# caki35/UNet-Torch

Hardware: AMD Instinct MI355X
Metric: images/sec training step, 4-level U-Net 1ch→2cls 512×512, at 1/2/4/8 MI355X (higher is better)
Workload: dtype f16

## Files before the change

unet-torch_amd/csrc/stem_head.hip:

```cpp
#include "kernels.h"

typedef _Float16 half8 __attribute__((ext_vector_type(8)));

namespace {

constexpr int STEM_PPB = 1024;
constexpr int WG_PPB = 4096;

inline bool al16(const void* p) { return (((uintptr_t)p) & 15) == 0; }

template <int CI>
__global__ __launch_bounds__(256) void stem3x3_fwd_kernel(const half_t* __restrict__ x, int ldx,
                                                          const float4* __restrict__ tx, const half_t* __restrict__ wp,
                                                          half_t* __restrict__ y, int ldy, float* __restrict__ part,
                                                          int N, int H, int W, int Co) {
    extern __shared__ __attribute__((aligned(16))) float sm[];
    const int tid = threadIdx.x;
    const int G = Co >> 3, PL = 256 / G;
    const int cg = tid % G, pl = tid / G;
    float* wsm = sm;
    for (int i = tid; i < 9 * CI * Co; i += 256) wsm[i] = (float)wp[i];
    __syncthreads();
    const long P = (long)N * H * W;
    const long p0 = (long)blockIdx.x * STEM_PPB;
    float s[8], q[8];
#pragma unroll
    for (int j = 0; j < 8; ++j) s[j] = q[j] = 0.f;
    const int RUN = STEM_PPB / PL;
    long p = p0 + (long)pl * RUN;
    long pend = p + RUN;
    if (pend > P) pend = P;
    if (pend > p0 + STEM_PPB) pend = p0 + STEM_PPB;
    int n = 0, yy = 0, xx = 0;
    if (p < pend) {
        n = (int)(p / ((long)H * W));
        const int r = (int)(p - (long)n * H * W);
        yy = r / W;
        xx = r - yy * W;
    }
    float win[3][3][CI];
    bool fresh = true;
    for (; p < pend; ++p) {
#pragma unroll
        for (int dy = 0; dy < 3; ++dy) {
            const int hi = yy + dy - 1;
            const bool rowok = hi >= 0 && hi < H;
            const half_t* xr = x + ((long)((long)n * H + (rowok ? hi : 0)) * W) * ldx;
#pragma unroll
            for (int dx = 0; dx < 3; ++dx) {
                if (!fresh && dx < 2) {
#pragma unroll
                    for (int ci = 0; ci < CI; ++ci) win[dy][dx][ci] = win[dy][dx + 1][ci];
                    continue;
                }
                const int wi = xx + dx - 1;
                const bool ok = rowok && wi >= 0 && wi < W;
#pragma unroll
                for (int ci = 0; ci < CI; ++ci) {
                    float v = 0.f;
                    if (ok) {
                        v = (float)xr[(long)wi * ldx + ci];
                        if (tx) v = umi_tx(v, tx[ci]);
                    }
                    win[dy][dx][ci] = v;
                }
            }
        }
        fresh = false;
        float acc[8];
#pragma unroll
        for (int j = 0; j < 8; ++j) acc[j] = 0.f;
#pragma unroll
        for (int tap = 0; tap < 9; ++tap)
#pragma unroll
            for (int ci = 0; ci < CI; ++ci) {
                const float v = win[tap / 3][tap % 3][ci];
                const float4* wrow = reinterpret_cast<const float4*>(wsm + (tap * CI + ci) * Co + cg * 8);
                float4 w0 = wrow[0], w1 = wrow[1];
                acc[0] = fmaf(v, w0.x, acc[0]); acc[1] = fmaf(v, w0.y, acc[1]);
                acc[2] = fmaf(v, w0.z, acc[2]); acc[3] = fmaf(v, w0.w, acc[3]);
                acc[4] = fmaf(v, w1.x, acc[4]); acc[5] = fmaf(v, w1.y, acc[5]);
                acc[6] = fmaf(v, w1.z, acc[6]); acc[7] = fmaf(v, w1.w, acc[7]);
            }
        half8 o;
#pragma unroll
        for (int j = 0; j < 8; ++j) {
            o[j] = (half_t)acc[j];
            float vr = (float)o[j];
            s[j] += vr;
            q[j] = fmaf(vr, vr, q[j]);
        }
        *reinterpret_cast<half8*>(y + p * ldy + cg * 8) = o;
        if (++xx == W) {
            xx = 0;
            fresh = true;
            if (++yy == H) { yy = 0; ++n; }
        }
    }
    if (part) {
        __syncthreads();
        float* red = sm;
#pragma unroll
        for (int j = 0; j < 8; ++j) { red[(0 * 256 + tid) * 9 + j] = s[j]; red[(1 * 256 + tid) * 9 + j] = q[j]; }
        __syncthreads();
        for (int i = tid; i < 2 * Co; i += 256) {
            int which = i / Co, c = i - which * Co;
            float a = 0.f;
            for (int k = 0; k < PL; ++k) a += red[(which * 256 + k * G + (c >> 3)) * 9 + (c & 7)];
            part[((long)blockIdx.x * 2 + which) * Co + c] = a;
        }
    }
}

struct StemBna { const half_t* y; int ldy; const float4* tx; const float* rstd; const float* sum_dz; const float* sum_dzx; long M; };

template <bool BNA>
__global__ __launch_bounds__(256) void stem3x3_wgrad_kernel(const half_t* __restrict__ x, int ldx,
                                                            const float4* __restrict__ tx,
                                                            const half_t* __restrict__ dy, int lddy,
                                                            float* __restrict__ part, int N, int H, int W, int Ci,
                                                            int Co, StemBna ba) {
    __shared__ float red[256][9];
    const int tid = threadIdx.x, ci = blockIdx.y;
    const int G = Co >> 3, PL = 256 / G;
    const int cg = tid % G, pl = tid / G;
    const long P = (long)N * H * W;
    const long p0 = (long)blockIdx.x * WG_PPB;
    float acc[9][8];
#pragma unroll
    for (int t = 0; t < 9; ++t)
#pragma unroll
        for (int j = 0; j < 8; ++j) acc[t][j] = 0.f;
    float4 tc = tx ? tx[ci] : make_float4(0.f, 1.f, 0.f, -INFINITY);
    float4 tb[BNA ? 8 : 1];
    float rsb[BNA ? 8 : 1], c1[BNA ? 8 : 1], c2[BNA ? 8 : 1];
    if (BNA) {
        const float invM = 1.f / (float)ba.M;
#pragma unroll
        for (int j = 0; j < 8; ++j) {
            const int c = cg * 8 + j;
            tb[j] = ba.tx[c];
            rsb[j] = ba.rstd[c];
            c1[j] = ba.sum_dz[c] * invM;
            c2[j] = ba.sum_dzx[c] * invM;
        }
    }
    long p = p0 + pl;
    long pend = p0 + WG_PPB;
    if (pend > P) pend = P;
    int n = 0, yy = 0, xx = 0;
    if (p < pend) {
        n = (int)(p / ((long)H * W));
        const int r = (int)(p - (long)n * H * W);
        yy = r / W;
        xx = r - yy * W;
    }
#pragma unroll 4
    for (; p < pend; p += PL) {
        const half8 g = *reinterpret_cast<const half8*>(dy + p * lddy + cg * 8);
        float win[9];
#pragma unroll
        for (int dy_ = 0; dy_ < 3; ++dy_) {
            const int hi = yy + dy_ - 1;
            const bool rowok = hi >= 0 && hi < H;
            const half_t* xr = x + ((long)((long)n * H + (rowok ? hi : 0)) * W) * ldx + ci;
#pragma unroll
            for (int dx = 0; dx < 3; ++dx) {
                const int wi = xx + dx - 1;
                const bool ok = rowok && wi >= 0 && wi < W;
                float v = (float)xr[(long)(ok ? wi : 0) * ldx];
                if (tx) v = umi_tx(v, tc);
                win[dy_ * 3 + dx] = ok ? v : 0.f;
            }
        }
        float gf[8];
        if (BNA) {
            const half8 yv = *reinterpret_cast<const half8*>(ba.y + p * ba.ldy + cg * 8);
#pragma unroll
            for (int j = 0; j < 8; ++j) gf[j] = (float)umi_bn_dz<_Float16>((float)yv[j], (float)g[j], tb[j], rsb[j], c1[j], c2[j]);
        } else {
#pragma unroll
            for (int j = 0; j < 8; ++j) gf[j] = (float)g[j];
        }
#pragma unroll
        for (int tap = 0; tap < 9; ++tap)
#pragma unroll
            for (int j = 0; j < 8; ++j) acc[tap][j] = fmaf(win[tap], gf[j], acc[tap][j]);
        xx += PL;
        while (xx >= W) {
            xx -= W;
            if (++yy == H) { yy = 0; ++n; }
        }
    }
    for (int tap = 0; tap < 9; ++tap) {
        __syncthreads();
#pragma unroll
        for (int j = 0; j < 8; ++j) red[tid][j] = acc[tap][j];
        __syncthreads();
        if (tid < Co) {
            float a = 0.f;
            for (int k = 0; k < PL; ++k) a += red[k * G + (tid >> 3)][tid & 7];
            part[(((long)blockIdx.x * 9 + tap) * Ci + ci) * Co + tid] = a;
        }
    }
}

template <int NC, typename TO, bool STATS>
__global__ __launch_bounds__(256) void head1x1_fwd_kernel(const half_t* __restrict__ x, int ldx,
                                                          const float4* __restrict__ tx, const half_t* __restrict__ wp,
                                                          const float* __restrict__ bias, TO* __restrict__ y, int ldy,
                                                          float* __restrict__ part, long P, int C) {
    const int G = C >> 3;
    const long gt = (long)blockIdx.x * 256 + threadIdx.x;
    const int cg = (int)(gt % G);
    const long stride_p = ((long)gridDim.x * 256) / G;
    float4 t[8];
    float w[8][NC];
#pragma unroll
    for (int j = 0; j < 8; ++j) {
        t[j] = tx ? tx[cg * 8 + j] : make_float4(0.f, 1.f, 0.f, -INFINITY);
#pragma unroll
        for (int k = 0; k < NC; ++k) w[j][k] = (float)wp[(cg * 8 + j) * NC + k];
    }
    float ssum[NC], ssq[NC];
#pragma unroll
    for (int k = 0; k < NC; ++k) ssum[k] = ssq[k] = 0.f;
    const long Pr = ((P + stride_p - 1) / stride_p) * stride_p;
    for (long p = gt / G; p < Pr; p += stride_p) {
        float acc[NC];
#pragma unroll
        for (int k = 0; k < NC; ++k) acc[k] = 0.f;
        if (p < P) {
            half8 v = *reinterpret_cast<const half8*>(x + p * ldx + cg * 8);
#pragma unroll
            for (int j = 0; j < 8; ++j) {
                float a = umi_tx((float)v[j], t[j]);
#pragma unroll
                for (int k = 0; k < NC; ++k) acc[k] = fmaf(a, w[j][k], acc[k]);
            }
        }
        for (int o = G >> 1; o > 0; o >>= 1)
#pragma unroll
            for (int k = 0; k < NC; ++k) acc[k] += __shfl_xor(acc[k], o);
        if (cg == 0 && p < P) {
#pragma unroll
            for (int k = 0; k < NC; ++k) {
                const TO o = (TO)(acc[k] + (bias ? bias[k] : 0.f));
                y[p * ldy + k] = o;
                if (STATS) {
                    const float vr = (float)o;
                    ssum[k] += vr;
                    ssq[k] = fmaf(vr, vr, ssq[k]);
                }
            }
        }
    }
    if (STATS) {
        __shared__ float red[4][2][NC];
#pragma unroll
        for (int k = 0; k < NC; ++k)
            for (int o = 32; o > 0; o >>= 1) {
                ssum[k] += __shfl_xor(ssum[k], o);
                ssq[k] += __shfl_xor(ssq[k], o);
            }
        if ((threadIdx.x & 63) == 0) {
#pragma unroll
            for (int k = 0; k < NC; ++k) {
                red[threadIdx.x >> 6][0][k] = ssum[k];
                red[threadIdx.x >> 6][1][k] = ssq[k];
            }
        }
        __syncthreads();
        if (threadIdx.x < 2 * NC) {
            const int which = threadIdx.x / NC, k = threadIdx.x - which * NC;
            part[((long)blockIdx.x * 2 + which) * NC + k] =
                (red[0][which][k] + red[1][which][k]) + (red[2][which][k] + red[3][which][k]);
        }
    }
}

template <int NC>
__global__ __launch_bounds__(256) void smallk1x1_fwd_kernel(const half_t* __restrict__ x, int ldx,
                                                            const half_t* __restrict__ wp, half_t* __restrict__ y,
                                                            int ldy, long P, int C) {
    const int G = C >> 3;
    const long gt = (long)blockIdx.x * 256 + threadIdx.x;
// ... 87 lines not shown
                float a = 0.f;
                for (int qq = 0; qq < 256 / G; ++qq) a += red[0][qq * G + (threadIdx.x >> 3)][threadIdx.x & 7];
                wpart[((long)blockIdx.x * C + threadIdx.x) * NC + k] = a;
            }
        }
    }
}

template <int NC>
__global__ __launch_bounds__(256) void head1x1_wgrad_kernel(const half_t* __restrict__ x, int ldx,
                                                            const float4* __restrict__ tx,
                                                            const half_t* __restrict__ dl, int lddl,
                                                            float* __restrict__ part, long P, int C, int ppb) {
    __shared__ float red[256][9];
    const int tid = threadIdx.x;
    const int G = C >> 3, PL = 256 / G;
    const int cg = tid % G, pl = tid / G;
    const long p0 = (long)blockIdx.x * ppb;
    float4 t[8];
#pragma unroll
    for (int j = 0; j < 8; ++j) t[j] = tx ? tx[cg * 8 + j] : make_float4(0.f, 1.f, 0.f, -INFINITY);
    float acc[NC][8];
#pragma unroll
    for (int k = 0; k < NC; ++k)
#pragma unroll
        for (int j = 0; j < 8; ++j) acc[k][j] = 0.f;
    for (long p = p0 + pl; p < p0 + ppb && p < P; p += PL) {
        half8 v = *reinterpret_cast<const half8*>(x + p * ldx + cg * 8);
        float a[8];
#pragma unroll
        for (int j = 0; j < 8; ++j) a[j] = umi_tx((float)v[j], t[j]);
#pragma unroll
        for (int k = 0; k < NC; ++k) {
            float d = (float)dl[p * lddl + k];
#pragma unroll
            for (int j = 0; j < 8; ++j) acc[k][j] = fmaf(a[j], d, acc[k][j]);
        }
    }
    for (int k = 0; k < NC; ++k) {
        __syncthreads();
#pragma unroll
        for (int j = 0; j < 8; ++j) red[tid][j] = acc[k][j];
        __syncthreads();
        if (tid < C) {
            float s = 0.f;
            for (int q = 0; q < PL; ++q) s += red[q * G + (tid >> 3)][tid & 7];
            part[((long)blockIdx.x * C + tid) * NC + k] = s;
        }
    }
}

__global__ __launch_bounds__(256) void head_wpart_reduce_kernel(const float* __restrict__ wpart, int rows, int C, int NC,
                                                                float* __restrict__ dW, long s_co, long s_ci, float scale) {
    __shared__ double sh[256];
    const int e = blockIdx.x, tid = threadIdx.x;
    double a = 0.0;
    for (int r = tid; r < rows; r += 256) a += (double)wpart[(long)r * C * NC + e];
    sh[tid] = a;
    __syncthreads();
    for (int o = 128; o > 0; o >>= 1) {
        if (tid < o) sh[tid] += sh[tid + o];
        __syncthreads();
    }
    if (tid == 0) dW[(e % NC) * s_co + (e / NC) * s_ci] = (float)(sh[0] * (double)scale);
}

int grid_for(long items) {
    long g = (items + 255) / 256;
    if (g > 8192) g = 8192;
    return g < 1 ? 1 : (int)g;
}

bool groups_ok(int C) { return C % 8 == 0 && C / 8 <= 64 && (256 % (C / 8)) == 0; }

}

bool umi_stem_fwd_ok(const ConvFwdProblem& p) {
    if (p.flags & (UMI_CONV_UPSAMPLE2 | UMI_CONV_FORCE_GENERIC)) return false;
    return p.in_dtype == UMI_F16 && p.out_dtype == UMI_F16 && !p.has_bias && p.R == 3 && p.S == 3 && p.stride == 1 && p.pad == 1 &&
           p.Ci >= 1 && p.Ci <= 4 && groups_ok(p.Co) && p.ldy % 8 == 0 && 9 * p.Ci * p.Co * 4 <= 48 * 1024;
}
int umi_stem_stat_rows(int N, int H, int W) { return (int)(((long)N * H * W + STEM_PPB - 1) / STEM_PPB); }

int umi_stem_fwd(const ConvFwdProblem& p, const void* x, const void* tx, const void* wp, void* y, float* part, hipStream_t s) {
    if (!al16(y)) return UMI_ERR_BADARG;
    const int Ci = p.Ci, Co = p.Co;
    const int rows = umi_stem_stat_rows(p.N, p.H, p.W);
    size_t smem = (size_t)9 * Ci * Co * 4;
    if (smem < 2 * 256 * 9 * 4) smem = 2 * 256 * 9 * 4;
#define GO(CI) hipLaunchKernelGGL(stem3x3_fwd_kernel<CI>, dim3(rows), dim3(256), smem, s, (const half_t*)x, p.ldx, (const float4*)tx, (const half_t*)wp, (half_t*)y, p.ldy, part, p.N, p.H, p.W, Co)
    switch (Ci) { case 1: GO(1); break; case 2: GO(2); break; case 3: GO(3); break; default: GO(4); }
#undef GO
    UMI_LAUNCH_CHECK();
    return UMI_OK;
}

bool umi_stem_wgrad_ok(const WgradProblem& p) {
    if (p.flags & UMI_CONV_FORCE_GENERIC) return false;
    return p.dtype == UMI_F16 && !p.has_txb && p.R == 3 && p.S == 3 && p.stride == 1 && p.pad == 1 && p.Ci >= 1 && p.Ci <= 4 &&
           groups_ok(p.Co) && p.Co <= 256 && p.lddy % 8 == 0;
}
static size_t stem_wgrad_ws_bytes(long P, int Ci, int Co) {
    return (size_t)((P + WG_PPB - 1) / WG_PPB) * 9 * Ci * Co * sizeof(float);
}
size_t umi_stem_wgrad_ws_bound(const WgradProblem& facts) {
    WgradProblem p = facts;
    p.stride = p.pad = 1; p.ldx = p.lddy = 8;
    return umi_stem_wgrad_ok(p) ? stem_wgrad_ws_bytes((long)p.N * p.Ho * p.Wo, p.Ci, p.Co) : 0;
}
int umi_stem_wgrad(const WgradProblem& p, const void* x, const void* txa, const void* dy, const WgradOut& o, hipStream_t s,
                   const WgradBnApply* bna) {
    if (o.ws_bytes < stem_wgrad_ws_bytes((long)p.N * p.H * p.W, p.Ci, p.Co)) return UMI_ERR_WORKSPACE;
    if (!al16(dy) || (bna && !al16(bna->y))) return UMI_ERR_BADARG;
    const int N = p.N, H = p.H, W = p.W, Ci = p.Ci, Co = p.Co;
    int blocks = (int)(((long)N * H * W + WG_PPB - 1) / WG_PPB);
    if (!bna)
        hipLaunchKernelGGL(stem3x3_wgrad_kernel<false>, dim3(blocks, Ci), dim3(256), 0, s, (const half_t*)x, p.ldx, (const float4*)txa,
                           (const half_t*)dy, p.lddy, (float*)o.ws, N, H, W, Ci, Co, StemBna{});
    else {
        const StemBna ba{(const half_t*)bna->y, bna->ldy, (const float4*)bna->tx_bn, bna->rstd, bna->sum_dz, bna->sum_dzx, (long)N * H * W};
        hipLaunchKernelGGL(stem3x3_wgrad_kernel<true>, dim3(blocks, Ci), dim3(256), 0, s, (const half_t*)x, p.ldx, (const float4*)txa,
                           (const half_t*)dy, p.lddy, (float*)o.ws, N, H, W, Ci, Co, ba);
    }
    UMI_LAUNCH_CHECK();
    umi_launch_wgrad_reduce(blocks, 9, Ci, Co, o, s);
    UMI_LAUNCH_CHECK();
    return UMI_OK;
}

bool umi_head_fwd_ok(const ConvFwdProblem& p) {
    if (p.flags & (UMI_CONV_UPSAMPLE2 | UMI_CONV_FORCE_GENERIC)) return false;
    return p.in_dtype == UMI_F16 && (p.out_dtype == UMI_F32 || p.out_dtype == UMI_F16) && p.R == 1 && p.S == 1 && p.stride == 1 &&
           p.pad == 0 && p.Co >= 1 && p.Co <= 8 && groups_ok(p.Ci) && p.ldx % 8 == 0;
}
int umi_head_stat_rows(long P, int Ci) { return grid_for(P * (Ci / 8)); }
int umi_head_fwd(const ConvFwdProblem& p, const void* x, const void* tx, const void* wp, const float* bias, void* y, float* part,
                 hipStream_t s) {
    if (!al16(x)) return UMI_ERR_BADARG;
    const long P = (long)p.N * p.H * p.W;
    const int Ci = p.Ci, out_dtype = p.out_dtype;
    if (part && out_dtype != UMI_F16) return UMI_ERR_UNSUPPORTED;
    int grid = grid_for(P * (Ci / 8));
#define GO_(NC, TO, ST) hipLaunchKernelGGL((head1x1_fwd_kernel<NC, TO, ST>), dim3(grid), dim3(256), 0, s, (const half_t*)x, p.ldx, (const float4*)tx, (const half_t*)wp, bias, (TO*)y, p.ldy, part, P, Ci)
#define GO(NC)                                                          \
    do {                                                                \
        if (out_dtype == UMI_F32) GO_(NC, float, false);                \
        else if (part) GO_(NC, half_t, true);                           \
        else GO_(NC, half_t, false);                                    \
    } while (0)
    switch (p.Co) { case 1: GO(1); break; case 2: GO(2); break; case 3: GO(3); break; case 4: GO(4); break;
                    case 5: GO(5); break; case 6: GO(6); break; case 7: GO(7); break; default: GO(8); }
#undef GO
#undef GO_
    UMI_LAUNCH_CHECK();
    return UMI_OK;
}

bool umi_smallk_fwd_ok(const ConvFwdProblem& p) {
    if (p.flags & (UMI_CONV_UPSAMPLE2 | UMI_CONV_FORCE_GENERIC)) return false;
    return p.in_dtype == UMI_F16 && p.out_dtype == UMI_F16 && !p.has_tx && !p.has_bias && p.R == 1 && p.S == 1 && p.stride == 1 &&
           p.pad == 0 && p.Ci >= 1 && p.Ci <= 8 && groups_ok(p.Co) && p.ldy % 8 == 0;
}
int umi_smallk_fwd(const ConvFwdProblem& p, const void* x, const void* wp, void* y, hipStream_t s) {
    if (!al16(y)) return UMI_ERR_BADARG;
    const long P = (long)p.N * p.H * p.W;
    const int Co = p.Co;
    int grid = grid_for(P * (Co / 8));
#define GO(NC) hipLaunchKernelGGL(smallk1x1_fwd_kernel<NC>, dim3(grid), dim3(256), 0, s, (const half_t*)x, p.ldx, (const half_t*)wp, (half_t*)y, p.ldy, P, Co)
    switch (p.Ci) { case 1: GO(1); break; case 2: GO(2); break; case 3: GO(3); break; case 4: GO(4); break;
                    case 5: GO(5); break; case 6: GO(6); break; case 7: GO(7); break; default: GO(8); }
#undef GO
    UMI_LAUNCH_CHECK();
    return UMI_OK;
}

int umi_smallk_bnred_rows(long P, int Co) { return grid_for(P * (Co / 8)); }
int umi_smallk_fwd_bnred(const void* x, int ldx, const void* wp, void* y, int ldy, const void* ybn, int ldybn, const void* txbn,
                         const float* rstd, float* part, long P, int Ci, int Co, hipStream_t s, float* dW, long s_co, long s_ci,
                         float out_scale, void* ws, size_t ws_bytes) {
    if (!al16(y) || !al16(ybn)) return UMI_ERR_BADARG;
    int grid = grid_for(P * (Co / 8));
    float* wpart = nullptr;
    if (dW) {
        if (!ws || ws_bytes < (size_t)grid * Co * Ci * sizeof(float)) return UMI_ERR_WORKSPACE;
        wpart = (float*)ws;
    }
#define GO(NC) hipLaunchKernelGGL(smallk1x1_bnred_kernel<NC>, dim3(grid), dim3(256), 0, s, (const half_t*)x, ldx, (const half_t*)wp, (half_t*)y, ldy, (const half_t*)ybn, ldybn, (const float4*)txbn, rstd, part, P, Co, wpart)
    switch (Ci) { case 1: GO(1); break; case 2: GO(2); break; case 3: GO(3); break; case 4: GO(4); break;
                  case 5: GO(5); break; case 6: GO(6); break; case 7: GO(7); break; default: GO(8); }
#undef GO
    UMI_LAUNCH_CHECK();
    if (dW) {
        hipLaunchKernelGGL(head_wpart_reduce_kernel, dim3(Co * Ci), dim3(256), 0, s, (const float*)wpart, grid, Co, Ci, dW, s_co, s_ci,
                           out_scale);
        UMI_LAUNCH_CHECK();
    }
    return UMI_OK;
}

bool umi_head_wgrad_ok(const WgradProblem& p) {
    if (p.flags & UMI_CONV_FORCE_GENERIC) return false;
    return p.dtype == UMI_F16 && !p.has_txb && p.R == 1 && p.S == 1 && p.stride == 1 && p.pad == 0 && p.Co >= 1 && p.Co <= 8 &&
           groups_ok(p.Ci) && p.Ci <= 256 && p.ldx % 8 == 0;
}
static int head_wgrad_ppb(long P) {
    long ppb = (P + 2047) / 2048;
    ppb = ((ppb + 255) / 256) * 256;
    if (ppb > WG_PPB) ppb = WG_PPB;
// ... 27 lines not shown
```

Measured before the change: 743.9.

## Stage stem conv input windows in LDS and pipeline wgrad with persistent blocks

Adds a specialized single-input-channel stem forward kernel. It stages three input rows per block into LDS and slides a register window across them, using packed f32x2 FMAs. The stem weight-gradient kernel becomes persistent: a capped grid loops over slabs in 1024-pixel chunks. It double-buffers the x-window staging in LDS and prefetches dy (and y for the BN-apply path) through a 4-deep register ring. The aim is to cut redundant global gathers of the 3x3 neighbourhood and hide load latency, at the cost of more registers and LDS and more complex boundary handling.

After: 750.8, median of 6. About the same (+0.9%).

```diff
diff --git a/unet-torch_amd/csrc/stem_head.hip b/unet-torch_amd/csrc/stem_head.hip
--- a/unet-torch_amd/csrc/stem_head.hip
+++ b/unet-torch_amd/csrc/stem_head.hip
@@ -8,6 +8,184 @@
 constexpr int WG_PPB = 4096;
 
 inline bool al16(const void* p) { return (((uintptr_t)p) & 15) == 0; }
+
+typedef float f32x2 __attribute__((ext_vector_type(2)));
+__device__ __forceinline__ f32x2 stem_fma2(float a, f32x2 b, f32x2 c) {
+    return __builtin_elementwise_fma(f32x2{a, a}, b, c);
+}
+
+constexpr int ST_WG_WGS = 512;
+constexpr int ST_RING = 4;
+constexpr int ST_CHP = 1024;
+
+__device__ __forceinline__ void stem_coords(long p, long P, int H, int W, int& yy, int& xx) {
+    if (P < 0x7fff0000L) {
+        const unsigned r = (unsigned)p / (unsigned)W;
+        xx = (int)((unsigned)p - r * (unsigned)W);
+        yy = (int)(r % (unsigned)H);
+    } else {
+        const long r = p / W;
+        xx = (int)(p - r * W);
+        yy = (int)(r % H);
+    }
+}
+
+struct StemStaged { half_t v[4][3], h[3]; int flag[4]; };
+
+__device__ __forceinline__ void stem_stage_load(StemStaged& st, const half_t* __restrict__ x, int ldx, long pc, long P, int H, int W,
+                                                int tid) {
+    const long rs = (long)W * ldx;
+    int yy, xx;
+    stem_coords(pc + tid, P, H, W, yy, xx);
+#pragma unroll
+    for (int i = 0; i < 4; ++i) {
+        const long p = pc + i * 256 + tid;
+        const bool in = p < P;
+        const half_t* xc = x + (in ? p : 0) * ldx;
+        const bool edge = (i == 0 && tid == 0) || (i == 3 && tid == 255);
+        const long hoff = !in ? 0 : tid == 0 ? (xx > 0 ? -ldx : 0) : (xx < W - 1 ? ldx : 0);
+        int f = (xx == 0 ? 1 : 0) | (xx == W - 1 ? 2 : 0);
+#pragma unroll
+        for (int dy = 0; dy < 3; ++dy) {
+            const bool ok = in && (dy == 0 ? yy > 0 : dy == 2 ? yy < H - 1 : true);
+            const half_t* xr = xc + (ok ? (dy - 1) * rs : 0);
+            f |= ok ? 4 << dy : 0;
+            st.v[i][dy] = xr[0];
+            if (edge) st.h[dy] = xr[hoff];
+        }
+        st.flag[i] = f;
+        if (i < 3) {
+            xx += 256;
+            while (xx >= W) { xx -= W; if (++yy == H) yy = 0; }
+        }
+    }
+}
+
+__device__ __forceinline__ void stem_stage_store(const StemStaged& st, bool has_tx, const float4 t, float* win, int row, int sh,
+                                                 int* flag, int tid) {
+#pragma unroll
+    for (int i = 0; i < 4; ++i) {
+        const int n = i * 256 + tid + 1;
+#pragma unroll
+        for (int dy = 0; dy < 3; ++dy) {
+            float v = (float)st.v[i][dy];
+            if (has_tx) v = umi_tx(v, t);
+            win[dy * row + n + (n >> sh)] = st.flag[i] & (4 << dy) ? v : 0.f;
+        }
+        if (flag) flag[i * 256 + tid] = st.flag[i];
+    }
+    if (tid == 0 || tid == 255) {
+        const int n = tid == 0 ? 0 : ST_CHP + 1, f = st.flag[tid == 0 ? 0 : 3];
+#pragma unroll
+        for (int dy = 0; dy < 3; ++dy) {
+            float v = (float)st.h[dy];
+            if (has_tx) v = umi_tx(v, t);
+            win[dy * row + n + (n >> sh)] = f & (4 << dy) ? v : 0.f;
+        }
+    }
+}
+constexpr int ST_WG_ROW = ST_CHP + 2;
+constexpr int ST_WG_STG = 3 * ST_WG_ROW + ST_CHP + 2;
+
+__device__ __forceinline__ void stem_window(float (&v)[9], const float* win, int q) {
+    const int f = ((const int*)(win + 3 * ST_WG_ROW))[q];
+#pragma unroll
+    for (int dy = 0; dy < 3; ++dy)
+#pragma unroll
+        for (int dx = 0; dx < 3; ++dx) {
+            const float t = win[dy * ST_WG_ROW + q + dx];
+            v[dy * 3 + dx] = (dx == 0 && (f & 1)) || (dx == 2 && (f & 2)) ? 0.f : t;
+        }
+}
+
+constexpr int ST_F1_ROW = STEM_PPB + 2 + (STEM_PPB + 2) / 4 + 2;
+__global__ __launch_bounds__(256) __attribute__((amdgpu_waves_per_eu(3))) void stem3x3_fwd1_kernel(
+    const half_t* __restrict__ x, int ldx, const float4* __restrict__ tx, const half_t* __restrict__ wp, half_t* __restrict__ y, int ldy,
+    float* __restrict__ part, int N, int H, int W, int Co) {
+    extern __shared__ __attribute__((aligned(16))) float sm[];
+    const int tid = threadIdx.x;
+    const int G = Co >> 3, PL = 256 / G;
+    const int cg = tid % G, pl = tid / G;
+    const int RUN = STEM_PPB / PL, sh = __ffs(RUN) - 1;
+    const long P = (long)N * H * W;
+    const long p0 = (long)blockIdx.x * STEM_PPB;
+    StemStaged st;
+    stem_stage_load(st, x, ldx, p0, P, H, W, tid);
+    f32x2 wr[9][4];
+#pragma unroll
+    for (int k = 0; k < 9; ++k)
+#pragma unroll
+        for (int j = 0; j < 4; ++j) wr[k][j] = f32x2{(float)wp[k * Co + cg * 8 + 2 * j], (float)wp[k * Co + cg * 8 + 2 * j + 1]};
+    stem_stage_store(st, tx != nullptr, tx ? tx[0] : make_float4(0.f, 1.f, 0.f, -INFINITY), sm, ST_F1_ROW, sh, nullptr, tid);
+    __syncthreads();
+    f32x2 s[4], q[4];
+#pragma unroll
+    for (int j = 0; j < 4; ++j) s[j] = q[j] = f32x2{0.f, 0.f};
+    int li = pl * RUN;
+    long p = p0 + li;
+    long pend = p + RUN;
+    if (pend > P) pend = P;
+    int xx = 0;
+    if (p < pend) {
+        int yy;
+        stem_coords(p, P, H, W, yy, xx);
+    }
+    float r[3][3];
+#pragma unroll
+    for (int dy = 0; dy < 3; ++dy) {
+        r[dy][1] = sm[dy * ST_F1_ROW + li + (li >> sh)];
+        r[dy][2] = sm[dy * ST_F1_ROW + li + 1 + ((li + 1) >> sh)];
+    }
+#pragma unroll 2
+    for (; p < pend; ++p, ++li) {
+        const int n = li + 2;
+        const bool lout = xx == 0, rout = xx == W - 1;
+        float v[9];
+#pragma unroll
+        for (int dy = 0; dy < 3; ++dy) {
+            r[dy][0] = r[dy][1];
+            r[dy][1] = r[dy][2];
+            r[dy][2] = sm[dy * ST_F1_ROW + n + (n >> sh)];
+            v[dy * 3 + 0] = lout ? 0.f : r[dy][0];
+            v[dy * 3 + 1] = r[dy][1];
+            v[dy * 3 + 2] = rout ? 0.f : r[dy][2];
+        }
+        f32x2 acc[4];
+#pragma unroll
+        for (int j = 0; j < 4; ++j) acc[j] = f32x2{0.f, 0.f};
+#pragma unroll
+        for (int tap = 0; tap < 9; ++tap)
+#pragma unroll
+            for (int j = 0; j < 4; ++j) acc[j] = stem_fma2(v[tap], wr[tap][j], acc[j]);
+        half8 o;
+#pragma unroll
+        for (int j = 0; j < 4; ++j) {
+            o[2 * j] = (half_t)acc[j].x;
+            o[2 * j + 1] = (half_t)acc[j].y;
+            const f32x2 vr = f32x2{(float)o[2 * j], (float)o[2 * j + 1]};
+            s[j] += vr;
+            q[j] = __builtin_elementwise_fma(vr, vr, q[j]);
+        }
+        *reinterpret_cast<half8*>(y + p * ldy + cg * 8) = o;
+        if (++xx == W) xx = 0;
+    }
+    if (part) {
+        __syncthreads();
+        float* red = sm;
+#pragma unroll
+        for (int j = 0; j < 4; ++j) {
+            red[(0 * 256 + tid) * 9 + 2 * j] = s[j].x; red[(0 * 256 + tid) * 9 + 2 * j + 1] = s[j].y;
+            red[(1 * 256 + tid) * 9 + 2 * j] = q[j].x; red[(1 * 256 + tid) * 9 + 2 * j + 1] = q[j].y;
+        }
+        __syncthreads();
+        for (int i = tid; i < 2 * Co; i += 256) {
+            int which = i / Co, c = i - which * Co;
+            float a = 0.f;
+            for (int k = 0; k < PL; ++k) a += red[(which * 256 + k * G + (c >> 3)) * 9 + (c & 7)];
+            part[((long)blockIdx.x * 2 + which) * Co + c] = a;
+        }
+    }
+}
 
 template <int CI>
 __global__ __launch_bounds__(256) void stem3x3_fwd_kernel(const half_t* __restrict__ x, int ldx,
@@ -115,23 +293,79 @@
 struct StemBna { const half_t* y; int ldy; const float4* tx; const float* rstd; const float* sum_dz; const float* sum_dzx; long M; };
 
 template <bool BNA>
-__global__ __launch_bounds__(256) void stem3x3_wgrad_kernel(const half_t* __restrict__ x, int ldx,
-                                                            const float4* __restrict__ tx,
-                                                            const half_t* __restrict__ dy, int lddy,
-                                                            float* __restrict__ part, int N, int H, int W, int Ci,
-                                                            int Co, StemBna ba) {
-    __shared__ float red[256][9];
+struct StemRing { half8 g[ST_RING], y[BNA ? ST_RING : 1]; };
+struct StemLane { size_t g0, gstep, y0, ystep, cgb; };
+struct StemChunkAddr { const char* g; const char* y; size_t glim, ylim; };
+
+__device__ __forceinline__ StemChunkAddr stem_chunk_addr(const half_t* dy, int lddy, const half_t* y, int ldy, long pc, long P) {
+    constexpr long CHP = ST_CHP;
+    const long last = P - 1 - pc < CHP - 1 ? P - 1 - pc : CHP - 1;
+    return StemChunkAddr{(const char*)(dy + pc * lddy), (const char*)(y ? y + pc * ldy : nullptr), (size_t)(last * lddy * 2),
+                         (size_t)(last * ldy * 2)};
+}
+template <bool BNA>
+__device__ __forceinline__ void stem_ring_issue(StemRing<BNA>& rg, int u, const StemChunkAddr& ca, const StemLane& ln, int t) {
+    const size_t og = ln.g0 + (size_t)t * ln.gstep;
+    rg.g[u] = *reinterpret_cast<const half8*>(ca.g + ((og < ca.glim ? og : ca.glim) + ln.cgb));
+    if (BNA) {
+        const size_t oy = ln.y0 + (size_t)t * ln.ystep;
+        rg.y[u] = *reinterpret_cast<const half8*>(ca.y + ((oy < ca.ylim ? oy : ca.ylim) + ln.cgb));
+    }
+}
+
+template <bool BNA>
+__device__ __forceinline__ void stem_wgrad_chunk(f32x2 (&acc)[9][4], StemRing<BNA>& rg, const float* win, const StemChunkAddr& cu,
+                                                 const StemChunkAddr& nx, const StemLane& ln, int nvalid, int T, int PL, int pl,
+                                                 const float4* tb, const float* rsb, const float* c1, const float* c2) {
+    for (int t0 = 0; t0 < T; t0 += ST_RING) {
+        const bool wrap = t0 + ST_RING >= T;
+        const StemChunkAddr ra = wrap ? nx : cu;
+        const int tr = wrap ? t0 + ST_RING - T : t0 + ST_RING;
+#pragma unroll
+        for (int u = 0; u < ST_RING; ++u) {
+            const int q = (t0 + u) * PL + pl;
+            const half8 g = rg.g[u];
+            float gf[8];
+            if (BNA) {
+                const half8 yv = rg.y[u];
+#pragma unroll
+                for (int j = 0; j < 8; ++j) gf[j] = (float)umi_bn_dz<_Float16>((float)yv[j], (float)g[j], tb[j], rsb[j], c1[j], c2[j]);
+            } else {
+#pragma unroll
+                for (int j = 0; j < 8; ++j) gf[j] = (float)g[j];
+            }
+            stem_ring_issue<BNA>(rg, u, ra, ln, tr + u);
+            float v[9];
+            stem_window(v, win, q);
+            if (q < nvalid) {
+#pragma unroll
+                for (int tap = 0; tap < 9; ++tap)
+#pragma unroll
+                    for (int j = 0; j < 4; ++j) acc[tap][j] = stem_fma2(v[tap], f32x2{gf[2 * j], gf[2 * j + 1]}, acc[tap][j]);
+            }
+        }
+    }
+}
+
+template <bool BNA>
+__global__ __launch_bounds__(256) __attribute__((amdgpu_waves_per_eu(2))) void stem3x3_wgrad_kernel(
+    const half_t* __restrict__ x, int ldx, const float4* __restrict__ tx, const half_t* __restrict__ dy, int lddy, float* __restrict__ part,
+    int N, int H, int W, int Ci, int Co, int slabs, StemBna ba) {
+    extern __shared__ __attribute__((aligned(16))) float sm[];
+    constexpr int CHP = ST_CHP, STG = ST_WG_STG;
+    constexpr int CPB = WG_PPB / CHP;
     const int tid = threadIdx.x, ci = blockIdx.y;
     const int G = Co >> 3, PL = 256 / G;
     const int cg = tid % G, pl = tid / G;
+    const int T = 4 * G;
     const long P = (long)N * H * W;
-    const long p0 = (long)blockIdx.x * WG_PPB;
-    float acc[9][8];
+    f32x2 acc[9][4];
 #pragma unroll
     for (int t = 0; t < 9; ++t)
 #pragma unroll
-        for (int j = 0; j < 8; ++j) acc[t][j] = 0.f;
-    float4 tc = tx ? tx[ci] : make_float4(0.f, 1.f, 0.f, -INFINITY);
+        for (int j = 0; j < 4; ++j) acc[t][j] = f32x2{0.f, 0.f};
+    const bool has_tx = tx != nullptr;
+    const float4 tc = has_tx ? tx[ci] : make_float4(0.f, 1.f, 0.f, -INFINITY);
     float4 tb[BNA ? 8 : 1];
     float rsb[BNA ? 8 : 1], c1[BNA ? 8 : 1], c2[BNA ? 8 : 1];
     if (BNA) {
@@ -145,63 +379,52 @@
             c2[j] = ba.sum_dzx[c] * invM;
         }
     }
-    long p = p0 + pl;
-    long pend = p0 + WG_PPB;
-    if (pend > P) pend = P;
-    int n = 0, yy = 0, xx = 0;
-    if (p < pend) {
-        n = (int)(p / ((long)H * W));
-        const int r = (int)(p - (long)n * H * W);
-        yy = r / W;
-        xx = r - yy * W;
-    }
-#pragma unroll 4
-    for (; p < pend; p += PL) {
-        const half8 g = *reinterpret_cast<const half8*>(dy + p * lddy + cg * 8);
-        float win[9];
-#pragma unroll
-        for (int dy_ = 0; dy_ < 3; ++dy_) {
-            const int hi = yy + dy_ - 1;
-            const bool rowok = hi >= 0 && hi < H;
-            const half_t* xr = x + ((long)((long)n * H + (rowok ? hi : 0)) * W) * ldx + ci;
-#pragma unroll
-            for (int dx = 0; dx < 3; ++dx) {
-                const int wi = xx + dx - 1;
-                const bool ok = rowok && wi >= 0 && wi < W;
-                float v = (float)xr[(long)(ok ? wi : 0) * ldx];
-                if (tx) v = umi_tx(v, tc);
-                win[dy_ * 3 + dx] = ok ? v : 0.f;
-            }
-        }
-        float gf[8];
-        if (BNA) {
-            const half8 yv = *reinterpret_cast<const half8*>(ba.y + p * ba.ldy + cg * 8);
-#pragma unroll
-            for (int j = 0; j < 8; ++j) gf[j] = (float)umi_bn_dz<_Float16>((float)yv[j], (float)g[j], tb[j], rsb[j], c1[j], c2[j]);
-        } else {
-#pragma unroll
-            for (int j = 0; j < 8; ++j) gf[j] = (float)g[j];
-        }
-#pragma unroll
-        for (int tap = 0; tap < 9; ++tap)
-#pragma unroll
-            for (int j = 0; j < 8; ++j) acc[tap][j] = fmaf(win[tap], gf[j], acc[tap][j]);
-        xx += PL;
-        while (xx >= W) {
-            xx -= W;
-            if (++yy == H) { yy = 0; ++n; }
-        }
-    }
-    for (int tap = 0; tap < 9; ++tap) {
+    float* red = sm + 2 * STG;
+    const half_t* xi = x + ci;
+    StemStaged st;
+    StemRing<BNA> rg;
+    int r = blockIdx.x, c = 0, b = 0;
+    stem_stage_load(st, xi, ldx, (long)r * WG_PPB, P, H, W, tid);
+    const StemLane ln{(size_t)pl * lddy * 2, (size_t)PL * lddy * 2, (size_t)pl * ba.ldy * 2, (size_t)PL * ba.ldy * 2, (size_t)cg * 16};
+    StemChunkAddr cu = stem_chunk_addr(dy, lddy, ba.y, ba.ldy, (long)r * WG_PPB, P);
+#pragma unroll
+    for (int u = 0; u < ST_RING; ++u) stem_ring_issue<BNA>(rg, u, cu, ln, u);
+    stem_stage_store(st, has_tx, tc, sm, ST_WG_ROW, 31, (int*)(sm + 3 * ST_WG_ROW), tid);
+    __syncthreads();
+    for (;;) {
+        int rn = r, cn = c + 1;
+        if (cn == CPB) { cn = 0; rn = r + (int)gridDim.x; }
+        const long pc = (long)r * WG_PPB + c * CHP;
+        const long pnx = (long)rn * WG_PPB + cn * CHP;
+        const bool more = rn < slabs && pnx < P;
+        if (more) stem_stage_load(st, xi, ldx, pnx, P, H, W, tid);
+        const float* win = sm + b * STG;
+        const StemChunkAddr nx = more ? stem_chunk_addr(dy, lddy, ba.y, ba.ldy, pnx, P) : cu;
+        stem_wgrad_chunk<BNA>(acc, rg, win, cu, nx, ln, P - pc < CHP ? (int)(P - pc) : CHP, T, PL, pl, tb, rsb, c1, c2);
+        if (cn == 0 || !more) {
+            for (int tap = 0; tap < 9; ++tap) {
+                __syncthreads();
+#pragma unroll
+                for (int j = 0; j < 4; ++j) { red[tid * 9 + 2 * j] = acc[tap][j].x; red[tid * 9 + 2 * j + 1] = acc[tap][j].y; }
+                __syncthreads();
+                if (tid < Co) {
+                    float a = 0.f;
+                    for (int k = 0; k < PL; ++k) a += red[(k * G + (tid >> 3)) * 9 + (tid & 7)];
+                    part[(((long)r * 9 + tap) * Ci + ci) * Co + tid] = a;
+                }
+            }
+#pragma unroll
+            for (int t = 0; t < 9; ++t)
+#pragma unroll
+                for (int j = 0; j < 4; ++j) acc[t][j] = f32x2{0.f, 0.f};
+        }
+        if (!more) break;
+        cu = nx;
+        b ^= 1;
+        stem_stage_store(st, has_tx, tc, sm + b * STG, ST_WG_ROW, 31, (int*)(sm + b * STG + 3 * ST_WG_ROW), tid);
         __syncthreads();
-#pragma unroll
-        for (int j = 0; j < 8; ++j) red[tid][j] = acc[tap][j];
-        __syncthreads();
-        if (tid < Co) {
-            float a = 0.f;
-            for (int k = 0; k < PL; ++k) a += red[k * G + (tid >> 3)][tid & 7];
-            part[(((long)blockIdx.x * 9 + tap) * Ci + ci) * Co + tid] = a;
-        }
+        r = rn;
+        c = cn;
     }
 }
 
@@ -461,8 +684,15 @@
     const int rows = umi_stem_stat_rows(p.N, p.H, p.W);
     size_t smem = (size_t)9 * Ci * Co * 4;
     if (smem < 2 * 256 * 9 * 4) smem = 2 * 256 * 9 * 4;
+    if (Ci == 1) {
+        const size_t sm1 = 3 * ST_F1_ROW * 4 > 2 * 256 * 9 * 4 ? 3 * ST_F1_ROW * 4 : 2 * 256 * 9 * 4;
+        hipLaunchKernelGGL(stem3x3_fwd1_kernel, dim3(rows), dim3(256), sm1, s, (const half_t*)x, p.ldx, (const float4*)tx, (const half_t*)wp,
+                           (half_t*)y, p.ldy, part, p.N, p.H, p.W, Co);
+        UMI_LAUNCH_CHECK();
+        return UMI_OK;
+    }
 #define GO(CI) hipLaunchKernelGGL(stem3x3_fwd_kernel<CI>, dim3(rows), dim3(256), smem, s, (const half_t*)x, p.ldx, (const float4*)tx, (const half_t*)wp, (half_t*)y, p.ldy, part, p.N, p.H, p.W, Co)
-    switch (Ci) { case 1: GO(1); break; case 2: GO(2); break; case 3: GO(3); break; default: GO(4); }
+    switch (Ci) { case 2: GO(2); break; case 3: GO(3); break; default: GO(4); }
 #undef GO
     UMI_LAUNCH_CHECK();
     return UMI_OK;
@@ -486,17 +716,20 @@
     if (o.ws_bytes < stem_wgrad_ws_bytes((long)p.N * p.H * p.W, p.Ci, p.Co)) return UMI_ERR_WORKSPACE;
     if (!al16(dy) || (bna && !al16(bna->y))) return UMI_ERR_BADARG;
     const int N = p.N, H = p.H, W = p.W, Ci = p.Ci, Co = p.Co;
-    int blocks = (int)(((long)N * H * W + WG_PPB - 1) / WG_PPB);
+    const int slabs = (int)(((long)N * H * W + WG_PPB - 1) / WG_PPB);
+    const int wgs = slabs < ST_WG_WGS ? slabs : ST_WG_WGS;
+    const int splits = slabs;
+    const size_t smem = ((size_t)2 * ST_WG_STG + 256 * 9) * 4;
     if (!bna)
-        hipLaunchKernelGGL(stem3x3_wgrad_kernel<false>, dim3(blocks, Ci), dim3(256), 0, s, (const half_t*)x, p.ldx, (const float4*)txa,
-                           (const half_t*)dy, p.lddy, (float*)o.ws, N, H, W, Ci, Co, StemBna{});
+        hipLaunchKernelGGL(stem3x3_wgrad_kernel<false>, dim3(wgs, Ci), dim3(256), smem, s, (const half_t*)x, p.ldx, (const float4*)txa,
+                           (const half_t*)dy, p.lddy, (float*)o.ws, N, H, W, Ci, Co, slabs, StemBna{});
     else {
         const StemBna ba{(const half_t*)bna->y, bna->ldy, (const float4*)bna->tx_bn, bna->rstd, bna->sum_dz, bna->sum_dzx, (long)N * H * W};
-        hipLaunchKernelGGL(stem3x3_wgrad_kernel<true>, dim3(blocks, Ci), dim3(256), 0, s, (const half_t*)x, p.ldx, (const float4*)txa,
-                           (const half_t*)dy, p.lddy, (float*)o.ws, N, H, W, Ci, Co, ba);
+        hipLaunchKernelGGL(stem3x3_wgrad_kernel<true>, dim3(wgs, Ci), dim3(256), smem, s, (const half_t*)x, p.ldx, (const float4*)txa,
+                           (const half_t*)dy, p.lddy, (float*)o.ws, N, H, W, Ci, Co, slabs, ba);
     }
     UMI_LAUNCH_CHECK();
-    umi_launch_wgrad_reduce(blocks, 9, Ci, Co, o, s);
+    umi_launch_wgrad_reduce(splits, 9, Ci, Co, o, s);
     UMI_LAUNCH_CHECK();
     return UMI_OK;
 }
```

## Stage stem conv input windows in LDS and software-pipeline wgrad loads

Applied to the files above, without the earlier changes.

The stem 3x3 forward and wgrad kernels now stage the block's input window (with halo rows), transformed to f32, into shared memory when it fits an LDS budget. Taps are then read from LDS instead of repeated strided global half loads. The wgrad kernel also double-buffers dy/y loads with sched barriers, uses packed f32x2 FMAs, moves the BN-apply constants into LDS to save registers, and sets a 3-wave occupancy hint. A non-staged fallback batches its global loads. The larger LDS footprint may reduce occupancy, and an env var controls the budget.

Result: slower. 758.9 before, 748.0 after (-1.4%).

```diff
diff --git a/unet-torch_amd/csrc/stem_head.hip b/unet-torch_amd/csrc/stem_head.hip
--- a/unet-torch_amd/csrc/stem_head.hip
+++ b/unet-torch_amd/csrc/stem_head.hip
@@ -1,4 +1,5 @@
 #include "kernels.h"
+#include <stdlib.h>
 
 typedef _Float16 half8 __attribute__((ext_vector_type(8)));
 
@@ -9,7 +10,57 @@
 
 inline bool al16(const void* p) { return (((uintptr_t)p) & 15) == 0; }
 
-template <int CI>
+typedef float f32x2 __attribute__((ext_vector_type(2)));
+
+__device__ __forceinline__ unsigned ld_h16(const half_t* p) { return *reinterpret_cast<const unsigned short*>(p); }
+__device__ __forceinline__ float h16_f(unsigned r) { return (float)__builtin_bit_cast(half_t, (unsigned short)r); }
+
+template <bool PAD>
+__device__ __forceinline__ int win_at(int i) { return PAD ? i + (i >> 5) : i; }
+inline size_t win_bytes(long ppb, int W, int CI, bool pad) {
+    const long cnt = (ppb + 2L * W + 2) * CI;
+    return (size_t)(cnt + (pad ? (cnt >> 5) + 1 : 0)) * sizeof(float);
+}
+
+template <int CI, bool PAD>
+__device__ __forceinline__ void stage_window(const half_t* __restrict__ x, int ldx, const float4* __restrict__ tx, long lo, int cnt,
+                                             float* xs, int tid) {
+    constexpr int EB = CI == 1 ? 16 : CI == 2 ? 8 : 4;
+    float4 tc[CI];
+#pragma unroll
+    for (int ci = 0; ci < CI; ++ci) tc[ci] = tx ? tx[ci] : make_float4(0.f, 1.f, 0.f, -INFINITY);
+    for (int base = 0; base < cnt; base += 256 * EB) {
+        unsigned raw[EB][CI];
+#pragma unroll
+        for (int k = 0; k < EB; ++k) {
+            const int e = base + k * 256 + tid, ec = e < cnt ? e : cnt - 1;
+            const half_t* px = x + (lo + ec) * ldx;
+#pragma unroll
+            for (int ci = 0; ci < CI; ++ci) {
+                raw[k][ci] = 0;
+                if (base + k * 256 < cnt) raw[k][ci] = ld_h16(px + ci);
+            }
+        }
+#pragma unroll
+        for (int k = 0; k < EB; ++k)
+#pragma unroll
+            for (int ci = 0; ci < CI; ++ci) asm volatile("" : "+v"(raw[k][ci]));
+#pragma unroll
+        for (int k = 0; k < EB; ++k) {
+            const int e = base + k * 256 + tid;
+            if (e < cnt) {
+#pragma unroll
+                for (int ci = 0; ci < CI; ++ci) {
+                    float v = h16_f(raw[k][ci]);
+                    if (tx) v = umi_tx(v, tc[ci]);
+                    xs[win_at<PAD>(e * CI + ci)] = v;
+                }
+            }
+        }
+    }
+}
+
+template <int CI, bool STAGE>
 __global__ __launch_bounds__(256) void stem3x3_fwd_kernel(const half_t* __restrict__ x, int ldx,
                                                           const float4* __restrict__ tx, const half_t* __restrict__ wp,
                                                           half_t* __restrict__ y, int ldy, float* __restrict__ part,
@@ -19,10 +70,18 @@
     const int G = Co >> 3, PL = 256 / G;
     const int cg = tid % G, pl = tid / G;
     float* wsm = sm;
+    float* xs = sm + 9 * CI * Co;
+    const long P = (long)N * H * W;
+    const long p0 = (long)blockIdx.x * STEM_PPB;
+    long lo = p0 - W - 1, hi = p0 + STEM_PPB + W + 1;
+    if (lo < 0) lo = 0;
+    if (hi > P) hi = P;
+    if (STAGE) stage_window<CI, true>(x, ldx, tx, lo, (int)(hi - lo), xs, tid);
     for (int i = tid; i < 9 * CI * Co; i += 256) wsm[i] = (float)wp[i];
     __syncthreads();
-    const long P = (long)N * H * W;
-    const long p0 = (long)blockIdx.x * STEM_PPB;
+    float4 tc[CI];
+#pragma unroll
+    for (int ci = 0; ci < CI; ++ci) tc[ci] = (!STAGE && tx) ? tx[ci] : make_float4(0.f, 1.f, 0.f, -INFINITY);
     float s[8], q[8];
 #pragma unroll
     for (int j = 0; j < 8; ++j) s[j] = q[j] = 0.f;
@@ -38,14 +97,39 @@
         yy = r / W;
         xx = r - yy * W;
     }
+    int rel = (int)(p - lo);
     float win[3][3][CI];
     bool fresh = true;
-    for (; p < pend; ++p) {
+    for (; p < pend; ++p, ++rel) {
+        unsigned raw[3][3][CI];
+        if (!STAGE) {
+#pragma unroll
+            for (int dy = 0; dy < 3; ++dy) {
+                const int hi_ = yy + dy - 1;
+                const bool rowok = hi_ >= 0 && hi_ < H;
+#pragma unroll
+                for (int dx = 0; dx < 3; ++dx) {
+                    const int wi = xx + dx - 1;
+                    const bool ok = rowok && wi >= 0 && wi < W;
+                    const half_t* px = x + (ok ? p + (long)(dy - 1) * W + (dx - 1) : p) * ldx;
+#pragma unroll
+                    for (int ci = 0; ci < CI; ++ci) {
+                        raw[dy][dx][ci] = 0;
+                        if (fresh || dx == 2) raw[dy][dx][ci] = ld_h16(px + ci);
+                    }
+                }
+            }
+#pragma unroll
+            for (int dy = 0; dy < 3; ++dy)
+#pragma unroll
+                for (int dx = 0; dx < 3; ++dx)
+#pragma unroll
+                    for (int ci = 0; ci < CI; ++ci) asm volatile("" : "+v"(raw[dy][dx][ci]));
+        }
 #pragma unroll
         for (int dy = 0; dy < 3; ++dy) {
-            const int hi = yy + dy - 1;
-            const bool rowok = hi >= 0 && hi < H;
-            const half_t* xr = x + ((long)((long)n * H + (rowok ? hi : 0)) * W) * ldx;
+            const int hi_ = yy + dy - 1;
+            const bool rowok = hi_ >= 0 && hi_ < H;
 #pragma unroll
             for (int dx = 0; dx < 3; ++dx) {
                 if (!fresh && dx < 2) {
@@ -55,14 +139,17 @@
                 }
                 const int wi = xx + dx - 1;
                 const bool ok = rowok && wi >= 0 && wi < W;
+                const int at = (ok ? rel + (dy - 1) * W + (dx - 1) : rel) * CI;
 #pragma unroll
                 for (int ci = 0; ci < CI; ++ci) {
-                    float v = 0.f;
-                    if (ok) {
-                        v = (float)xr[(long)wi * ldx + ci];
-                        if (tx) v = umi_tx(v, tx[ci]);
+                    float v;
+                    if (STAGE) {
+                        v = xs[win_at<true>(at + ci)];
+                    } else {
+                        v = h16_f(raw[dy][dx][ci]);
+                        if (tx) v = umi_tx(v, tc[ci]);
                     }
-                    win[dy][dx][ci] = v;
+                    win[dy][dx][ci] = ok ? v : 0.f;
                 }
             }
         }
@@ -114,88 +201,132 @@
 
 struct StemBna { const half_t* y; int ldy; const float4* tx; const float* rstd; const float* sum_dz; const float* sum_dzx; long M; };
 
-template <bool BNA>
-__global__ __launch_bounds__(256) void stem3x3_wgrad_kernel(const half_t* __restrict__ x, int ldx,
+template <bool BNA, bool STAGE>
+__global__ __launch_bounds__(256, 3) void stem3x3_wgrad_kernel(const half_t* __restrict__ x, int ldx,
                                                             const float4* __restrict__ tx,
                                                             const half_t* __restrict__ dy, int lddy,
                                                             float* __restrict__ part, int N, int H, int W, int Ci,
                                                             int Co, StemBna ba) {
-    __shared__ float red[256][9];
+    extern __shared__ __attribute__((aligned(16))) float sm[];
     const int tid = threadIdx.x, ci = blockIdx.y;
     const int G = Co >> 3, PL = 256 / G;
     const int cg = tid % G, pl = tid / G;
     const long P = (long)N * H * W;
     const long p0 = (long)blockIdx.x * WG_PPB;
-    float acc[9][8];
-#pragma unroll
-    for (int t = 0; t < 9; ++t)
-#pragma unroll
-        for (int j = 0; j < 8; ++j) acc[t][j] = 0.f;
-    float4 tc = tx ? tx[ci] : make_float4(0.f, 1.f, 0.f, -INFINITY);
-    float4 tb[BNA ? 8 : 1];
-    float rsb[BNA ? 8 : 1], c1[BNA ? 8 : 1], c2[BNA ? 8 : 1];
+    long lo = p0 - W - 1, hi = p0 + WG_PPB + W + 1;
+    if (lo < 0) lo = 0;
+    if (hi > P) hi = P;
+    float4* tbs = reinterpret_cast<float4*>(sm + (STAGE ? (WG_PPB + 2 * W + 2 + 3) & ~3 : 0));
+    float4* cbs = tbs + Co;
+    if (STAGE) stage_window<1, false>(x + ci, ldx, tx ? tx + ci : nullptr, lo, (int)(hi - lo), sm, tid);
     if (BNA) {
         const float invM = 1.f / (float)ba.M;
-#pragma unroll
-        for (int j = 0; j < 8; ++j) {
-            const int c = cg * 8 + j;
-            tb[j] = ba.tx[c];
-            rsb[j] = ba.rstd[c];
-            c1[j] = ba.sum_dz[c] * invM;
-            c2[j] = ba.sum_dzx[c] * invM;
-        }
-    }
+        for (int c = tid; c < Co; c += 256) {
+            tbs[c] = ba.tx[c];
+            cbs[c] = make_float4(ba.rstd[c], ba.sum_dz[c] * invM, ba.sum_dzx[c] * invM, 0.f);
+        }
+    }
+    if (STAGE || BNA) __syncthreads();
+    f32x2 acc[9][4];
+#pragma unroll
+    for (int t = 0; t < 9; ++t)
+#pragma unroll
+        for (int j = 0; j < 4; ++j) acc[t][j] = f32x2{0.f, 0.f};
+    float4 tc = tx ? tx[ci] : make_float4(0.f, 1.f, 0.f, -INFINITY);
     long p = p0 + pl;
     long pend = p0 + WG_PPB;
     if (pend > P) pend = P;
-    int n = 0, yy = 0, xx = 0;
+    int yy = 0, xx = 0;
     if (p < pend) {
-        n = (int)(p / ((long)H * W));
-        const int r = (int)(p - (long)n * H * W);
+        const int r = (int)(p % ((long)H * W));
         yy = r / W;
         xx = r - yy * W;
     }
-#pragma unroll 4
-    for (; p < pend; p += PL) {
-        const half8 g = *reinterpret_cast<const half8*>(dy + p * lddy + cg * 8);
+    const int sq = PL / W, sx = PL - sq * W, sy = sq % H;
+    int rel = (int)(p - lo);
+    auto fetch = [&](long pp, half8& g, half8& yv) {
+        if (pp >= pend) pp -= PL;
+#ifdef UMI_EXP_STEM_WG_NO_STREAM
+        asm volatile("" : "+v"(g), "+v"(yv));
+        return;
+#endif
+        g = *reinterpret_cast<const half8*>(dy + pp * lddy + cg * 8);
+        if (BNA) yv = *reinterpret_cast<const half8*>(ba.y + pp * ba.ldy + cg * 8);
+    };
+    auto trip = [&](const half8& g, const half8& yv) {
         float win[9];
 #pragma unroll
         for (int dy_ = 0; dy_ < 3; ++dy_) {
-            const int hi = yy + dy_ - 1;
-            const bool rowok = hi >= 0 && hi < H;
-            const half_t* xr = x + ((long)((long)n * H + (rowok ? hi : 0)) * W) * ldx + ci;
+            const int hi_ = yy + dy_ - 1;
+            const bool rowok = hi_ >= 0 && hi_ < H;
 #pragma unroll
             for (int dx = 0; dx < 3; ++dx) {
                 const int wi = xx + dx - 1;
                 const bool ok = rowok && wi >= 0 && wi < W;
-                float v = (float)xr[(long)(ok ? wi : 0) * ldx];
-                if (tx) v = umi_tx(v, tc);
+                const int off = (dy_ - 1) * W + (dx - 1);
+                float v;
+                if (STAGE) {
+                    v = sm[ok ? rel + off : rel];
+                } else {
+                    v = h16_f(ld_h16(x + (ok ? p + off : p) * ldx + ci));
+                    if (tx) v = umi_tx(v, tc);
+                }
                 win[dy_ * 3 + dx] = ok ? v : 0.f;
             }
         }
-        float gf[8];
+#ifdef UMI_EXP_STEM_WG_NO_MATH
+#pragma unroll
+        for (int t = 0; t < 9; ++t) asm volatile("" ::"v"(win[t]));
+        asm volatile("" ::"v"(g), "v"(yv));
+#else
+        f32x2 gf[4];
         if (BNA) {
-            const half8 yv = *reinterpret_cast<const half8*>(ba.y + p * ba.ldy + cg * 8);
-#pragma unroll
-            for (int j = 0; j < 8; ++j) gf[j] = (float)umi_bn_dz<_Float16>((float)yv[j], (float)g[j], tb[j], rsb[j], c1[j], c2[j]);
+            int opaque = 0;
+            asm volatile("" : "+v"(opaque));
+            const float4* tb = tbs + cg * 8 + opaque;
+            const float4* cb = cbs + cg * 8 + opaque;
+#pragma unroll
+            for (int j = 0; j < 8; ++j) {
+                const float4 c = cb[j];
+                gf[j >> 1][j & 1] = (float)umi_bn_dz<_Float16>((float)yv[j], (float)g[j], tb[j], c.x, c.y, c.z);
+            }
         } else {
 #pragma unroll
-            for (int j = 0; j < 8; ++j) gf[j] = (float)g[j];
-        }
-#pragma unroll
-        for (int tap = 0; tap < 9; ++tap)
-#pragma unroll
-            for (int j = 0; j < 8; ++j) acc[tap][j] = fmaf(win[tap], gf[j], acc[tap][j]);
-        xx += PL;
-        while (xx >= W) {
-            xx -= W;
-            if (++yy == H) { yy = 0; ++n; }
-        }
-    }
+            for (int j = 0; j < 8; ++j) gf[j >> 1][j & 1] = (float)g[j];
+        }
+#pragma unroll
+        for (int tap = 0; tap < 9; ++tap) {
+            const f32x2 w2 = {win[tap], win[tap]};
+#pragma unroll
+            for (int j = 0; j < 4; ++j) acc[tap][j] = __builtin_elementwise_fma(w2, gf[j], acc[tap][j]);
+        }
+#endif
+        p += PL;
+        rel += PL;
+        xx += sx;
+        const int carry = xx >= W ? 1 : 0;
+        xx -= carry ? W : 0;
+        yy += sy + carry;
+        yy -= yy >= H ? H : 0;
+    };
+    half8 gA = {}, yA = {}, gB = {}, yB = {};
+    if (p < pend) fetch(p, gA, yA);
+#pragma nounroll
+    while (p + PL < pend) {
+        fetch(p + PL, gB, yB);
+        __builtin_amdgcn_sched_barrier(0);
+        trip(gA, yA);
+        fetch(p + PL, gA, yA);
+        __builtin_amdgcn_sched_barrier(0);
+        trip(gB, yB);
+    }
+    if (p < pend) trip(gA, yA);
+    float (*red)[9] = reinterpret_cast<float (*)[9]>(sm);
+#pragma unroll
     for (int tap = 0; tap < 9; ++tap) {
         __syncthreads();
 #pragma unroll
-        for (int j = 0; j < 8; ++j) red[tid][j] = acc[tap][j];
+        for (int j = 0; j < 8; ++j) red[tid][j] = acc[tap][j >> 1][j & 1];
         __syncthreads();
         if (tid < Co) {
             float a = 0.f;
@@ -455,15 +586,29 @@
 }
 int umi_stem_stat_rows(int N, int H, int W) { return (int)(((long)N * H * W + STEM_PPB - 1) / STEM_PPB); }
 
+static size_t stem_lds_budget() {
+    const size_t most = 64 * 1024;
+    if (const char* e = getenv("UMI_STEM_LDS_BUDGET")) {
+        const long v = atol(e);
+        if (v >= 0 && (size_t)v < most) return (size_t)v;
+    }
+    return most;
+}
+
 int umi_stem_fwd(const ConvFwdProblem& p, const void* x, const void* tx, const void* wp, void* y, float* part, hipStream_t s) {
     if (!al16(y)) return UMI_ERR_BADARG;
     const int Ci = p.Ci, Co = p.Co;
     const int rows = umi_stem_stat_rows(p.N, p.H, p.W);
     size_t smem = (size_t)9 * Ci * Co * 4;
+    const size_t staged = smem + win_bytes(STEM_PPB, p.W, Ci, true);
+    const bool stage = staged <= stem_lds_budget();
+    if (stage) smem = staged;
     if (smem < 2 * 256 * 9 * 4) smem = 2 * 256 * 9 * 4;
-#define GO(CI) hipLaunchKernelGGL(stem3x3_fwd_kernel<CI>, dim3(rows), dim3(256), smem, s, (const half_t*)x, p.ldx, (const float4*)tx, (const half_t*)wp, (half_t*)y, p.ldy, part, p.N, p.H, p.W, Co)
+#define GO_(CI, ST) hipLaunchKernelGGL((stem3x3_fwd_kernel<CI, ST>), dim3(rows), dim3(256), smem, s, (const half_t*)x, p.ldx, (const float4*)tx, (const half_t*)wp, (half_t*)y, p.ldy, part, p.N, p.H, p.W, Co)
+#define GO(CI) do { if (stage) GO_(CI, true); else GO_(CI, false); } while (0)
     switch (Ci) { case 1: GO(1); break; case 2: GO(2); break; case 3: GO(3); break; default: GO(4); }
 #undef GO
+#undef GO_
     UMI_LAUNCH_CHECK();
     return UMI_OK;
 }
@@ -487,14 +632,16 @@
     if (!al16(dy) || (bna && !al16(bna->y))) return UMI_ERR_BADARG;
     const int N = p.N, H = p.H, W = p.W, Ci = p.Ci, Co = p.Co;
     int blocks = (int)(((long)N * H * W + WG_PPB - 1) / WG_PPB);
-    if (!bna)
-        hipLaunchKernelGGL(stem3x3_wgrad_kernel<false>, dim3(blocks, Ci), dim3(256), 0, s, (const half_t*)x, p.ldx, (const float4*)txa,
-                           (const half_t*)dy, p.lddy, (float*)o.ws, N, H, W, Ci, Co, StemBna{});
-    else {
-        const StemBna ba{(const half_t*)bna->y, bna->ldy, (const float4*)bna->tx_bn, bna->rstd, bna->sum_dz, bna->sum_dzx, (long)N * H * W};
-        hipLaunchKernelGGL(stem3x3_wgrad_kernel<true>, dim3(blocks, Ci), dim3(256), 0, s, (const half_t*)x, p.ldx, (const float4*)txa,
-                           (const half_t*)dy, p.lddy, (float*)o.ws, N, H, W, Ci, Co, ba);
-    }
+    size_t smem = ((win_bytes(WG_PPB, W, 1, false) + 15) & ~(size_t)15) + (size_t)Co * 32;
+    const bool stage = smem <= stem_lds_budget();
+    if (!stage) smem = (size_t)Co * 32;
+    if (smem < 256 * 9 * 4) smem = 256 * 9 * 4;
+    const StemBna ba = bna ? StemBna{(const half_t*)bna->y, bna->ldy, (const float4*)bna->tx_bn, bna->rstd, bna->sum_dz, bna->sum_dzx, (long)N * H * W}
+                           : StemBna{};
+#define GO(BN, ST) hipLaunchKernelGGL((stem3x3_wgrad_kernel<BN, ST>), dim3(blocks, Ci), dim3(256), smem, s, (const half_t*)x, p.ldx, (const float4*)txa, (const half_t*)dy, p.lddy, (float*)o.ws, N, H, W, Ci, Co, ba)
+    if (!bna) { if (stage) GO(false, true); else GO(false, false); }
+    else { if (stage) GO(true, true); else GO(true, false); }
+#undef GO
     UMI_LAUNCH_CHECK();
     umi_launch_wgrad_reduce(blocks, 9, Ci, Co, o, s);
     UMI_LAUNCH_CHECK();
```
